# mstksg/tensor-ops

Hardware: AMD Instinct MI355X
Metric: gradTOp steps/sec (ffLayer MNIST 784->256->10) + gmul TFLOP/s vs roofline (higher is better)
Workload: dtype f32

## Files before the change

tensor-ops_amd/csrc/gemm_small.hip:

```cpp
#include "common.hpp"

#include <type_traits>

namespace to {

typedef float f32x16 __attribute__((ext_vector_type(16)));

template <class S>
struct SmallArgsT {
  const S* A;
  const S* B;
  S* C;
  const S* Cin;
  int M, N, K;
  long a_sm, a_sk, b_sk, b_sn, c_sm;
  long a_sb, b_sb, c_sb;
  int a_vec, b_vec;
  unsigned a_bytes, b_bytes;
  int tiles_n;
  int tiles_m;
  int tile_order;
  int kper;
  S alpha, beta;
  const S* bias;
// ... 26 lines not shown
template <class G>
__device__ __forceinline__ void tile_of(const G& g, int bid, int& tile_m, int& tile_n) {
  if (g.tile_order) {
    const int T = g.tiles_m * g.tiles_n, x = bid & 7, q = T >> 3, r = T & 7;
    bid = (x < r ? x * (q + 1) : r * (q + 1) + (x - r) * q) + (bid >> 3);
  }
  if (g.tile_order == 2) {
    tile_n = bid / g.tiles_m;
    tile_m = bid - tile_n * g.tiles_m;
  } else {
    tile_m = bid / g.tiles_n;
    tile_n = bid - tile_m * g.tiles_n;
  }
}

__device__ __forceinline__ float tanh_s(float x) { return tanhf(x); }
__device__ __forceinline__ double tanh_s(double x) { return tanh(x); }
__device__ __forceinline__ float exp_s(float x) { return expf(x); }
__device__ __forceinline__ double exp_s(double x) { return exp(x); }
__device__ __forceinline__ float log_s(float x) { return logf(x); }
__device__ __forceinline__ double log_s(double x) { return log(x); }
__device__ __forceinline__ float max_s(float a, float b) { return fmaxf(a, b); }
__device__ __forceinline__ double max_s(double a, double b) { return fmax(a, b); }

template <class S, int AMODE, int BMODE, int NW, int TS, int ONESHOT = 0, bool EXT = false, int PARTS = 0, bool STAG = false>
__device__ __forceinline__ void gemm_small_body(const SmallArgsT<S>& g, const int bid, const long bz, S* ext_lds = nullptr,
                                                const int tid_in = -1) {
  constexpr int ES = (int)sizeof(S);
  static_assert(ES == 4 || TS == 16, "the fp64 matrix instruction is 16x16x4");
  constexpr int KG = (TS == 32) ? 2 : 4;
  constexpr int NR = (TS == 32) ? 16 : 4;
  constexpr int CK = 4 * KG;
  typedef S accv __attribute__((ext_vector_type(NR)));
  S (*red)[NR][64];
  S (*rsum)[64];
  S* dzs;
  if constexpr (EXT) {
    red = reinterpret_cast<S (*)[NR][64]>(ext_lds);
    rsum = reinterpret_cast<S (*)[64]>(ext_lds + NW * NR * 64);
    dzs = ext_lds + NW * NR * 64 + NW * 64;
  } else {
    __shared__ S red_s[NW][NR][64];
    __shared__ S rsum_s[NW][64];
    __shared__ S dzs_s[TS == 16 ? 16 * 17 : 1];
    red = red_s;
    rsum = rsum_s;
    dzs = dzs_s;
  }
  const int tid = tid_in >= 0 ? tid_in : (int)threadIdx.x, lane = tid & 63, wave = tid >> 6;
  const int l31 = lane & (TS - 1), half = lane / TS;
#ifdef TOPS_AB_KNOBS
  const bool stamp_on = g.dbg && bid == 0 && tid == 0;
#endif
  SM_STAMP(0);
  int tile_m, tile_n;
// ... 95 lines not shown
  };
  auto mma_part = [&](auto part) {
    constexpr int p = decltype(part)::value;
#pragma unroll
    for (int c = p * CP; c < (p + 1) * CP; ++c) {
#pragma unroll
      for (int j = 0; j < 4; ++j) {
        if constexpr (ES == 8) acc = __builtin_amdgcn_mfma_f64_16x16x4f64(a0[c][j], b0[c][j], acc, 0, 0, 0);
        else if constexpr (TS == 32) acc = __builtin_amdgcn_mfma_f32_32x32x2f32(a0[c][j], b0[c][j], acc, 0, 0, 0);
        else acc = __builtin_amdgcn_mfma_f32_16x16x4f32(a0[c][j], b0[c][j], acc, 0, 0, 0);
      }
      __builtin_amdgcn_sched_barrier(0);
#pragma unroll
      for (int j = 0; j < 4; ++j) asum += a0[c][j];
      __builtin_amdgcn_sched_barrier(0);
    }
  };
  auto row16 = [&](int kg, int r) { return ES == 8 ? kg + 4 * r : 4 * kg + r; };
  constexpr int NRW = (NR + NW - 1) / NW;
  S* Cb = g.C + bz * g.c_sb;
  const S* Ci = g.Cin ? g.Cin + bz * g.c_sb : nullptr;
  const S* Hd = g.dact ? g.dact + bz * g.c_sb : nullptr;
  S pf_ci[NRW], pf_hd[NRW], pf_bias = S(0);
  {
    const long col = (long)tile_n * TS + l31;
    if (g.bias && col < g.N) pf_bias = g.bias[col];
#pragma unroll
    for (int i = 0; i < NRW; ++i) {
      const int r = wave + i * NW;
      const int lrow = (TS == 32) ? (r & 3) + 8 * (r >> 2) + 4 * half : row16(half, r);
      const long row = (long)tile_m * TS + lrow;
      const bool ok = r < NR && row < g.M && col < g.N;
      pf_ci[i] = (Ci && ok) ? Ci[row * g.c_sm + col] : S(0);
      pf_hd[i] = (Hd && ok) ? Hd[row * g.c_sm + col] : S(0);
    }
  }
  constexpr int SK = CK * ST;
  SM_STAMP(1);
  if constexpr (ONESHOT) {
    if constexpr (PARTS == 0) {
      if (kbeg < kend) {
        load_stage(a0, b0, kbeg);
#ifdef TOPS_AB_KNOBS
        if (stamp_on) { SM_STAMP(2); __builtin_amdgcn_s_waitcnt(0x0F70); SM_STAMP(3); }
#endif
        mma_stage(a0, b0);
      }
    } else if (kbeg < kend) {
      if constexpr (STAG) {
        const int lvl = __builtin_amdgcn_readfirstlane(wave) >> 2;
        if (lvl == 0) __builtin_amdgcn_s_setprio(3);
        else if (lvl == 1) __builtin_amdgcn_s_setprio(2);
        else if (lvl == 2) __builtin_amdgcn_s_setprio(1);
      }
      load_part(std::integral_constant<int, 0>{}, kbeg);
      auto stage = [&](auto part) {
        constexpr int p = decltype(part)::value;
// ... 10 lines not shown
      if constexpr (PARTS > 2) stage(std::integral_constant<int, 2>{});
      if constexpr (PARTS > 3) stage(std::integral_constant<int, 3>{});
      if constexpr (PARTS > 4) {
        stage(std::integral_constant<int, 4>{});
        stage(std::integral_constant<int, 5>{});
        stage(std::integral_constant<int, 6>{});
        stage(std::integral_constant<int, 7>{});
      }
      static_assert(PARTS == 1 || PARTS == 2 || PARTS == 4 || PARTS == 8, "one, two, four or eight parts");
    }
  } else {
    S a1[ST][4], b1[ST][4];
    if (kbeg < kend) load_stage(a0, b0, kbeg);
    for (int k0 = kbeg; k0 < kend; k0 += 2 * SK) {
      if (k0 + SK < kend) load_stage(a1, b1, k0 + SK);
      mma_stage(a0, b0);
      if (k0 + SK < kend) {
        if (k0 + 2 * SK < kend) load_stage(a0, b0, k0 + 2 * SK);
        mma_stage(a1, b1);
      }
    }
  }

  S tl_bw[2][4], tl_hv[2][4];
  if constexpr (TS == 16) {
    if (g.loss_rows && g.tail_out) {
      const int l15 = lane & 15, kg = lane >> 4;
      const int ntiles = (g.tail_n + 15) / 16;
#pragma unroll
      for (int u = 0; u < 2; ++u) {
        const int t = wave + u * NW;
        const long col = (long)t * 16 + l15;
        const bool cv = t < ntiles && col < g.tail_n;
#pragma unroll
        for (int st = 0; st < 4; ++st) {
          const int k = 4 * st + kg;
          tl_bw[u][st] = (cv && k < g.N) ? g.tail_w[(long)k * g.tail_n + col] : S(0);
        }
#pragma unroll
        for (int r = 0; r < 4; ++r) {
          const long row = (long)tile_m * 16 + row16(kg, r);
          tl_hv[u][r] = (cv && row < g.M) ? g.tail_h[row * g.tail_n + col] : S(0);
        }
      }
    }
  }
#pragma unroll
  for (int r = 0; r < NR; ++r) red[wave][r][lane] = acc[r];
  rsum[wave][lane] = asum;
  SM_STAMP(4);
  __syncthreads();
  SM_STAMP(5);
  if (g.rowsum && tile_n == 0 && wave == 0 && lane < TS) {
    S v = S(0);
#pragma unroll
    for (int w = 0; w < NW; ++w)
#pragma unroll
      for (int q = 0; q < KG; ++q) v += rsum[w][lane + q * TS];
    const long row = (long)tile_m * TS + lane;
    if (row < g.M) g.rowsum[bz * g.M + row] = g.rowsum_acc ? g.rowsum_in[bz * g.M + row] + g.rowsum_alpha * v : v;
  }
#pragma unroll
  for (int i = 0; i < NRW; ++i) {
    const int r = wave + i * NW;
    if (r >= NR) break;
    S v = S(0);
#pragma unroll
    for (int w = 0; w < NW; ++w) v += red[w][r][lane];
    const int lrow = (TS == 32) ? (r & 3) + 8 * (r >> 2) + 4 * half : row16(half, r);
    const long row = (long)tile_m * TS + lrow;
    const long col = (long)tile_n * TS + l31;
    if constexpr (TS == 16) {
      if (g.loss_rows) {
        const bool valid = row < g.M && col < g.N;
        v = v * g.alpha + pf_bias;
        const S t = valid ? g.target[row * g.c_sm + col] : S(0);
        auto sum16 = [](S x) {
#pragma unroll
          for (int off = 8; off > 0; off >>= 1) x += __shfl_xor(x, off, 64);
          return x;
        };
        S out, l;
        if (g.loss_rows == 1) {
          S mx = valid ? v : S(-INFINITY);
#pragma unroll
          for (int off = 8; off > 0; off >>= 1) mx = max_s(mx, __shfl_xor(mx, off, 64));
          const S e = valid ? exp_s(v - mx) : S(0);
          const S se = sum16(e), sy = sum16(t);
          const S pr = e / se;
          out = pr * sy - t;
          l = valid ? -t * log_s(pr) : S(0);
        } else {
          const S sg = S(1) / (S(1) + exp_s(-v));
          const S e = t - sg;
          out = S(-2) * e * sg * (S(1) - sg);
          l = valid ? e * e : S(0);
        }
        if (valid) Cb[row * g.c_sm + col] = out;
        if (g.tail_out) dzs[lrow * 17 + l31] = valid ? out : S(0);
        if (g.loss_out) {
          l = sum16(l);
          if (l31 == 0 && row < g.M) g.loss_out[row] = l;
        }
        continue;
      }
    }
    if (row < g.M && col < g.N) {
      v *= g.alpha;
      if (Ci) v += g.beta * pf_ci[i];
      v += pf_bias;
      if (g.act == 1) v = S(1) / (S(1) + exp_s(-v));
      else if (g.act == 2) v = tanh_s(v);
      if (Hd) {
        const S h = pf_hd[i];
        v *= g.dact_kind ? S(1) - h * h : h * (S(1) - h);
      }
      Cb[row * g.c_sm + col] = v;
    }
  }
  SM_STAMP(6);
  if constexpr (TS == 16) {
    if (g.loss_rows && g.tail_out) {
      __syncthreads();
      typedef S acc4 __attribute__((ext_vector_type(4)));
      const int l15 = lane & 15, kg = lane >> 4;
      const int ntiles = (g.tail_n + 15) / 16;
      acc4 acc2[2];
#pragma unroll
      for (int u = 0; u < 2; ++u)
#pragma unroll
        for (int r = 0; r < 4; ++r) acc2[u][r] = S(0);
#pragma unroll
      for (int st = 0; st < 4; ++st) {
        if (4 * st < g.N) {
          const S a = dzs[l15 * 17 + 4 * st + kg];
#pragma unroll
          for (int u = 0; u < 2; ++u) {
            if constexpr (ES == 8) acc2[u] = __builtin_amdgcn_mfma_f64_16x16x4f64(a, tl_bw[u][st], acc2[u], 0, 0, 0);
            else acc2[u] = __builtin_amdgcn_mfma_f32_16x16x4f32(a, tl_bw[u][st], acc2[u], 0, 0, 0);
          }
        }
      }
#pragma unroll
      for (int u = 0; u < 2; ++u) {
        const int t = wave + u * NW;
        const long col = (long)t * 16 + l15;
#pragma unroll
        for (int r = 0; r < 4; ++r) {
          const long row = (long)tile_m * 16 + row16(kg, r);
          if (t < ntiles && row < g.M && col < g.tail_n)
            g.tail_out[row * g.tail_n + col] = acc2[u][r] * tl_hv[u][r] * (S(1) - tl_hv[u][r]);
        }
      }
      SM_STAMP(7);
    }
  }
#ifdef TOPS_AB_KNOBS
  if (stamp_on) { __builtin_amdgcn_s_waitcnt(0); SM_STAMP(8); }
#endif
}

template <class S, int AMODE, int BMODE, int NW, int TS, int ONESHOT = 0>
__global__ __launch_bounds__(NW * 64) void gemm_small_kernel(SmallArgsT<S> g) {
  gemm_small_body<S, AMODE, BMODE, NW, TS, ONESHOT>(g, (int)blockIdx.x, (long)blockIdx.z);
}

template <class S, int A1, int B1, int NW1, int TS1, int OS1, int A2, int B2, int NW2, int TS2, int OS2, int P1 = 0, bool STAG1 = false>
__global__ __launch_bounds__((NW1 > NW2 ? NW1 : NW2) * 64) void gemm_small_pair_kernel(SmallArgsT<S> g1,
                                                                                         SmallArgsT<S> g2, int n1) {
  if ((int)blockIdx.x < n1) {
    if (NW1 < NW2 && (int)(threadIdx.x >> 6) >= NW1) return;
    gemm_small_body<S, A1, B1, NW1, TS1, OS1, false, P1, STAG1>(g1, (int)blockIdx.x, 0);
  } else {
    if (NW2 < NW1 && (int)(threadIdx.x >> 6) >= NW2) return;
    gemm_small_body<S, A2, B2, NW2, TS2, OS2>(g2, (int)blockIdx.x - n1, 0);
  }
}

struct ChainSync {
  unsigned* ctr;
  int* status;
  long long timeout;
  int dev;
};

__device__ __forceinline__ bool chain_barrier(const ChainSync& cs, int which, unsigned epoch) {
  __shared__ int ok;
  if (cs.dev == 1) {
    __syncthreads();
    return true;
  }
  if (cs.dev != 2) __builtin_amdgcn_fence(__ATOMIC_RELEASE, "agent");
  if (threadIdx.x == 0) ok = 1;
  __syncthreads();
  unsigned* flags = cs.ctr + which * 256;
  if (threadIdx.x == 0) __hip_atomic_store(flags + blockIdx.x, epoch, __ATOMIC_RELEASE, __HIP_MEMORY_SCOPE_AGENT);
  if (threadIdx.x < gridDim.x) {
    const long long t0 = wall_clock64();
// ... 316 lines not shown
  const int tiles_m = (int)((p.M + TS - 1) / TS);
  g.tiles_n = (int)((p.N + TS - 1) / TS);
  g.tiles_m = tiles_m;
  g.tile_order = pick_tile_order(p, TS, g.tiles_m, g.tiles_n);
  dim3 grid(tiles_m * g.tiles_n, 1, (unsigned)p.batch), block(NW * 64);
  switch (amode * 2 + bmode) {
    case 0: launch_k((gemm_small_kernel<S, 0, 0, NW, TS, ONESHOT>), grid, block, 0, s, g); break;
    case 1: launch_k((gemm_small_kernel<S, 0, 1, NW, TS, ONESHOT>), grid, block, 0, s, g); break;
    case 2: launch_k((gemm_small_kernel<S, 1, 0, NW, TS, ONESHOT>), grid, block, 0, s, g); break;
    default: launch_k((gemm_small_kernel<S, 1, 1, NW, TS, ONESHOT>), grid, block, 0, s, g); break;
  }
}

#ifdef TOPS_AB_KNOBS
static long long* small_stamps(int which) {
  static const int want = [] { const char* e = ab_getenv("TOPS_SMALL_STAMPS"); return e ? atoi(e) : 0; }();
  if (!want || want != which) return nullptr;
  static long long* buf = [] {
    long long* p = nullptr;
    if (hipHostMalloc(&p, 16 * sizeof(long long), hipHostMallocMapped) != hipSuccess) return (long long*)nullptr;
    for (int i = 0; i < 16; ++i) p[i] = 0;
    static long long* keep = p;
    atexit([] {
      static const char* names[9] = {"entry", "set-up done", "operand batch issued", "operand batch landed", "MFMAs done, partial in LDS",
                                     "all partials there (barrier)", "reduced + epilogue / loss head, stores issued", "tail done", "stores acknowledged"};
      std::fprintf(stderr, "[small stamps %d] tile 0, thread 0, us since its workgroup began:", want);
      for (int i = 1; i < 9; ++i)
        if (keep[i]) std::fprintf(stderr, "\n  %6.2f  %s", (keep[i] - keep[0]) * 0.01, names[i]);
      std::fprintf(stderr, "\n");
    });
    return p;
  }();
  long long* dev = nullptr;
  if (buf && hipHostGetDevicePointer(reinterpret_cast<void**>(&dev), buf, 0) != hipSuccess) dev = nullptr;
  return dev;
}
#endif

struct SmallPlan {
  int ts, nw, os;
  int amode, bmode;
  bool f64_t32;
};

template <class S>
static SmallPlan plan_small(const GemmProblem& p, SmallArgsT<S>& g) {
  constexpr bool F64 = sizeof(S) == 8;
  g = SmallArgsT<S>{};
  g.A = (const S*)p.A; g.B = (const S*)p.B; g.C = (S*)p.C;
  g.Cin = (p.beta != 0.0) ? (const S*)p.Cin : nullptr;
// ... 344 lines not shown
```

tensor-ops_amd/csrc/gemm_t32.hip:

```cpp
#include <cstdio>
#include <type_traits>

#include "common.hpp"

namespace to {

typedef float f32x16 __attribute__((ext_vector_type(16)));
typedef float f32x4 __attribute__((ext_vector_type(4)));

struct T32Args {
  const float* A;
  const float* B;
  float* C;
  const float* Cin;
  const float* bias;
  const float* dact;
  float* rowsum;
  const float* rowsum_in;
  unsigned long long* dbg;
  long a_sx, b_sx;
  long c_sm;
  int M, N, K;
  int tiles_m, tiles_n;
  int gm, gn;
  int act, dact_kind;
  int rowsum_acc;
  int pd;
  float alpha, beta;
  float rowsum_alpha;
};

__device__ __attribute__((aligned(16))) float g_t32_zero[4] = {0.f, 0.f, 0.f, 0.f};

constexpr int T32_BK = 32, T32_NS = 2, T32_NW = 4;
constexpr int T32_CTR = 4096;
constexpr int T32_STAGE = 2 * 32 * T32_BK;
constexpr int T32_WAVE = T32_NS * T32_STAGE;

__device__ __forceinline__ bool t32_tile_of(int tiles_m, int tiles_n, int gm, int gn, int bid, int& tm, int& tn) {
  const int x = bid & 7, local = bid >> 3, xm = x / gn, xn = x - xm * gn;
  const int r0 = tiles_m * xm / gm, r1 = tiles_m * (xm + 1) / gm, c0 = tiles_n * xn / gn, c1 = tiles_n * (xn + 1) / gn;
  const int w = c1 - c0;
  if (w <= 0 || local >= (r1 - r0) * w) return false;
  tm = r0 + local / w;
  tn = c0 + local - (local / w) * w;
  return true;
}

__device__ __forceinline__ int t32_key(int x) { return (x >> 1) & 7; }

template <bool AKC, bool BKC, bool ARAG = false, bool WT = false, int NW = T32_NW, int NS = T32_NS, bool EARLY = false>
__device__ __forceinline__ int gemm_t32_body(const T32Args& g, const int bid, float* smem) {
  constexpr int WAVE_F = NS * T32_STAGE;
  static_assert(WAVE_F >= 1024 + 64, "a wave's stage memory holds its partial tile and its row sums");
  static_assert(!ARAG || !AKC, "the dword form is for a row-contiguous A");
  constexpr int NA = ARAG ? 16 : 4, PER = NA + 4;
  const int tid = threadIdx.x, lane = tid & 63;
  const int wave = __builtin_amdgcn_readfirstlane(tid >> 6);
  const int l31 = lane & 31, half = lane >> 5;
  unsigned long long* const dbg = (g.dbg && tid == 0 && (bid == 0 || bid == (int)gridDim.x - 1)) ? g.dbg + (bid == 0 ? 0 : 8) : nullptr;
  auto stamp = [&](int i) { if (dbg) dbg[i] = __builtin_amdgcn_s_memrealtime(); };
  int tile_m, tile_n;
  if (!t32_tile_of(g.tiles_m, g.tiles_n, g.gm, g.gn, bid, tile_m, tile_n)) return -1;
  stamp(0);
  const int m0 = tile_m * 32, n0 = tile_n * 32;

  const int erow = tid >> 3, ec4 = (tid & 7) * 4;
  const long grow = m0 + erow, gcol = n0 + ec4;
  const bool evalid = (NW == 4 || tid < 256) && grow < g.M && gcol < g.N;
  f32x4 pf_ci = {0.f, 0.f, 0.f, 0.f}, pf_hd = {0.f, 0.f, 0.f, 0.f}, pf_bias = {0.f, 0.f, 0.f, 0.f};
  auto prefetch_epilogue = [&] {
    if (evalid) {
      if (g.Cin) pf_ci = *reinterpret_cast<const f32x4*>(g.Cin + grow * g.c_sm + gcol);
      if (g.dact) pf_hd = *reinterpret_cast<const f32x4*>(g.dact + grow * g.c_sm + gcol);
      if (g.bias) pf_bias = *reinterpret_cast<const f32x4*>(g.bias + gcol);
    }
  };
  if constexpr (!EARLY) prefetch_epilogue();

  const int U = (g.K + 15) / 16;
  const int k0 = (int)((long)U * wave / NW) * 16;
  int k1 = (int)((long)U * (wave + 1) / NW) * 16;
  if (k1 > g.K) k1 = g.K;
  const int nC = k1 > k0 ? (k1 - k0 + T32_BK - 1) / T32_BK : 0;

  typedef __attribute__((address_space(3))) void* lptr_t;
  float* wsm = smem + wave * WAVE_F;
  const unsigned lds_w = __builtin_amdgcn_readfirstlane((unsigned)(unsigned long)(lptr_t)wsm);

  const int lr = lane >> 3, ls = lane & 7;
  unsigned oa[4], ob[4];
  bool xa_ok = true, xb_ok = true;
#pragma unroll
  for (int p = 0; p < 4; ++p) {
    if constexpr (AKC) {
      long x = m0 + 8 * p + lr;
      if (x >= g.M) x = g.M - 1;
      oa[p] = (unsigned)((x * g.a_sx + 4 * (ls ^ t32_key(8 * p + lr))) * 4);
    } else {
      oa[p] = (unsigned)(((long)(8 * p + lr) * g.a_sx + m0 + 4 * ls) * 4);
    }
    if constexpr (BKC) {
      long x = n0 + 8 * p + lr;
      if (x >= g.N) x = g.N - 1;
      ob[p] = (unsigned)((x * g.b_sx + 4 * (ls ^ t32_key(8 * p + lr))) * 4);
    } else {
      ob[p] = (unsigned)(((long)(8 * p + lr) * g.b_sx + n0 + 4 * ls) * 4);
    }
  }
  if constexpr (!AKC) xa_ok = m0 + 4 * ls + 3 < g.M;
  if constexpr (!BKC) xb_ok = n0 + 4 * ls + 3 < g.N;
  const bool interior = !ARAG && (AKC || m0 + 32 <= g.M) && (BKC || n0 + 32 <= g.N);
  const long step_a = AKC ? T32_BK * 4L : T32_BK * g.a_sx * 4L, step_b = BKC ? T32_BK * 4L : T32_BK * g.b_sx * 4L;
  const char* sa = reinterpret_cast<const char*>(g.A) + (AKC ? (long)k0 * 4 : (long)k0 * g.a_sx * 4);
  const char* sb = reinterpret_cast<const char*>(g.B) + (BKC ? (long)k0 * 4 : (long)k0 * g.b_sx * 4);

#define T32_DMA(OFF, BASE) asm volatile("global_load_lds_dwordx4 %0, %1 offset:0" ::"v"(OFF), "s"(BASE) : "memory")
#define T32_DMA_V(PTR) asm volatile("global_load_lds_dwordx4 %0, off offset:0" ::"v"(PTR) : "memory")
  const long a_sx_l = g.a_sx;
  const int M_l = g.M;
  auto issue = [&, a_sx_l, M_l](int c) {
    const int seq = c;
    const int kc = k0 + c * T32_BK;
    const unsigned st = lds_w + (unsigned)(seq % NS) * (T32_STAGE * 4);
    const char* ba = sa + (long)c * step_a;
    const char* bb = sb + (long)c * step_b;
    const bool full = kc + T32_BK <= k1;
    if (full && interior) {
#pragma unroll
      for (int p = 0; p < 4; ++p) {
        asm volatile("s_mov_b32 m0, %0\n\ts_nop 0" ::"s"(st + p * 1024) : "memory");
        T32_DMA(oa[p], ba);
      }
#pragma unroll
      for (int p = 0; p < 4; ++p) {
        asm volatile("s_mov_b32 m0, %0\n\ts_nop 0" ::"s"(st + 4096 + p * 1024) : "memory");
        T32_DMA(ob[p], bb);
      }
    } else {
      const char* zero = reinterpret_cast<const char*>(g_t32_zero);
      if constexpr (ARAG) {
#pragma unroll
        for (int e = 0; e < 16; ++e) {
          const int kl = 2 * e + half;
          const bool ok = kc + kl < k1 && m0 + l31 < M_l;
          const char* src = ok ? ba + ((long)kl * a_sx_l + m0 + l31) * 4 : zero;
          asm volatile("s_mov_b32 m0, %0\n\ts_nop 0" ::"s"(st + e * 256) : "memory");
          asm volatile("global_load_lds_dword %0, off offset:0" ::"v"(src) : "memory");
        }
      } else {
#pragma unroll
        for (int p = 0; p < 4; ++p) {
          const bool ok = AKC ? (kc + 4 * (ls ^ t32_key(8 * p + lr)) < k1) : (kc + 8 * p + lr < k1 && xa_ok);
          const char* src = ok ? ba + oa[p] : zero;
          asm volatile("s_mov_b32 m0, %0\n\ts_nop 0" ::"s"(st + p * 1024) : "memory");
          T32_DMA_V(src);
        }
      }
#pragma unroll
      for (int p = 0; p < 4; ++p) {
        const bool ok = BKC ? (kc + 4 * (ls ^ t32_key(8 * p + lr)) < k1) : (kc + 8 * p + lr < k1 && xb_ok);
        const char* src = ok ? bb + ob[p] : zero;
        asm volatile("s_mov_b32 m0, %0\n\ts_nop 0" ::"s"(st + 4096 + p * 1024) : "memory");
        T32_DMA_V(src);
      }
    }
  };
#undef T32_DMA
#undef T32_DMA_V

  f32x16 acc;
#pragma unroll
  for (int r = 0; r < 16; ++r) acc[r] = 0.f;
  float asum = 0.f;
  const bool want_rs = g.rowsum != nullptr && tile_n == 0;

  const int PD = g.pd < NS ? g.pd : NS;
  const int pro = nC < PD ? nC : PD;
  if constexpr (EARLY) {
    if (pro > 0) issue(0);
    __builtin_amdgcn_sched_barrier(0);
    prefetch_epilogue();
    __builtin_amdgcn_sched_barrier(0);
    for (int c = 1; c < pro; ++c) issue(c);
  } else {
    for (int c = 0; c < pro; ++c) issue(c);
  }
  stamp(1);

  auto wait_landed = [&](int c) {
    const int newer = (nC - 1 - c) < (PD - 1) ? (nC - 1 - c) : (PD - 1);
    static_assert(3 * PER <= 63, "vmcnt is six bits");
    if (newer >= 3) asm volatile("s_waitcnt vmcnt(%0)" ::"n"(3 * PER) : "memory");
    else if (newer == 2) asm volatile("s_waitcnt vmcnt(%0)" ::"n"(2 * PER) : "memory");
    else if (newer == 1) asm volatile("s_waitcnt vmcnt(%0)" ::"n"(PER) : "memory");
    else asm volatile("s_waitcnt vmcnt(0)" ::: "memory");
  };
  auto steps_of = [&](int c) { return (k1 - (k0 + c * T32_BK)) > 16 ? 4 : 2; };
  auto read_frags = [&](int c, float (&fa)[16], float (&fb)[16]) {
    const float* sp = wsm + (c % NS) * T32_STAGE;
    const int nI = steps_of(c);
#pragma unroll
    for (int i = 0; i < 4; ++i) {
      if (i < nI) {
        if constexpr (AKC) {
          const f32x4 v = *reinterpret_cast<const f32x4*>(sp + l31 * 32 + 4 * ((2 * i + half) ^ t32_key(l31)));
          fa[4 * i] = v.x; fa[4 * i + 1] = v.y; fa[4 * i + 2] = v.z; fa[4 * i + 3] = v.w;
        } else {
#pragma unroll
          for (int j = 0; j < 4; ++j) fa[4 * i + j] = sp[(4 * (2 * i + half) + j) * 32 + l31];
        }
        if constexpr (BKC) {
          const f32x4 v = *reinterpret_cast<const f32x4*>(sp + 1024 + l31 * 32 + 4 * ((2 * i + half) ^ t32_key(l31)));
          fb[4 * i] = v.x; fb[4 * i + 1] = v.y; fb[4 * i + 2] = v.z; fb[4 * i + 3] = v.w;
        } else {
#pragma unroll
          for (int j = 0; j < 4; ++j) fb[4 * i + j] = sp[1024 + (4 * (2 * i + half) + j) * 32 + l31];
        }
      }
    }
  };
  auto mma = [&](int c, const float (&fa)[16], const float (&fb)[16]) {
    const int nI = steps_of(c);
#pragma unroll
    for (int i = 0; i < 4; ++i) {
      if (i < nI) {
#pragma unroll
        for (int j = 0; j < 4; ++j) {
          acc = __builtin_amdgcn_mfma_f32_32x32x2f32(fa[4 * i + j], fb[4 * i + j], acc, 0, 0, 0);
          if (want_rs) asum += fa[4 * i + j];
        }
      }
    }
  };
  float fa[16], fb[16];
  for (int c = 0; c < nC; ++c) {
    wait_landed(c);
    if (c == 0) stamp(2);
    read_frags(c, fa, fb);
    asm volatile("s_waitcnt lgkmcnt(0)" ::: "memory");
    __builtin_amdgcn_sched_barrier(0);
    if (c + PD < nC) issue(c + PD);
    __builtin_amdgcn_sched_barrier(0);
    mma(c, fa, fb);
  }
  asm volatile("s_waitcnt vmcnt(0)" ::: "memory");
  stamp(3);

#pragma unroll
  for (int r = 0; r < 16; ++r) wsm[((r & 3) + 8 * (r >> 2) + 4 * half) * 32 + l31] = acc[r];
  if (want_rs) wsm[1024 + lane] = asum;
  __syncthreads();
  stamp(4);
  f32x4 s = {0.f, 0.f, 0.f, 0.f};
  if (NW == 4 || tid < 256) {
    s = *reinterpret_cast<const f32x4*>(smem + erow * 32 + ec4);
#pragma unroll
    for (int w = 1; w < NW; ++w) s += *reinterpret_cast<const f32x4*>(smem + w * WAVE_F + erow * 32 + ec4);
// ... 147 lines not shown
  if (hd) hd[3] = __builtin_amdgcn_s_memrealtime();
  if (h.tail_out) {
    f32x4 a = {0.f, 0.f, 0.f, 0.f};
#pragma unroll
    for (int n = 0; n < 16; ++n)
      if (n < h.N2) {
        const float d = __shfl(out_l, n, 64);
        a += w4[n] * d;
      }
    if (rv) *reinterpret_cast<f32x4*>(h.tail_out + grow * 256 + 4 * lane) = a * h4 * (1.f - h4);
  }
  if (hd) hd[4] = __builtin_amdgcn_s_memrealtime();
  __syncthreads();
  if (tid == 0) {
    unsigned* leave = h.ctr + T32_CTR + tile_m;
    const unsigned seen = __hip_atomic_fetch_add(leave, 1u, __ATOMIC_RELAXED, __HIP_MEMORY_SCOPE_AGENT);
    if (seen == (unsigned)(g.tiles_n - 1)) {
      __hip_atomic_store(h.ctr + tile_m, 0u, __ATOMIC_RELAXED, __HIP_MEMORY_SCOPE_AGENT);
      __hip_atomic_store(leave, 0u, __ATOMIC_RELAXED, __HIP_MEMORY_SCOPE_AGENT);
    }
  }
}

template <bool AKC, bool BKC, int NW = T32_NW, int NS = T32_NS, bool EARLY = false>
__global__ __launch_bounds__(NW * 64) void gemm_t32_kernel(T32Args g) {
  extern __shared__ __attribute__((aligned(1024))) float t32_smem[];
  gemm_t32_body<AKC, BKC, false, false, NW, NS, EARLY>(g, (int)blockIdx.x, t32_smem);
}

template <bool ARAG2>
__global__ __launch_bounds__(256) void gemm_t32_pair_kernel(T32Args g1, T32Args g2, int n1) {
  extern __shared__ __attribute__((aligned(1024))) float t32_smem[];
  if ((int)blockIdx.x < n1) gemm_t32_body<false, false, false>(g1, (int)blockIdx.x, t32_smem);
  else gemm_t32_body<false, false, ARAG2>(g2, (int)blockIdx.x - n1, t32_smem);
}

static bool t32_fill(const GemmProblem& p, T32Args& g, bool& akc, bool& bkc, bool allow_ragged_a = false, bool* ragged_a = nullptr) {
  if (p.dtype != TO_F32 || p.batch != 1 || p.reduce_batch) return false;
  if (p.loss_rows || p.tail_out || p.loss_out) return false;
  akc = p.a_sk == 1 && p.K > 1;
  bkc = p.b_sk == 1 && p.K > 1;
  if (!akc && p.a_sm != 1) return false;
  if (!bkc && p.b_sn != 1) return false;
  if (p.K % 4 != 0 || p.N % 4 != 0) return false;
  const bool rag = !akc && (p.M % 4 != 0 || p.a_sk % 4 != 0 || (reinterpret_cast<uintptr_t>(p.A) & 15u));
  if (ragged_a) *ragged_a = rag;
  if (rag && !allow_ragged_a) return false;
  if (akc && p.a_sm % 4 != 0) return false;
  if (bkc && p.b_sn % 4 != 0) return false;
  if (!bkc && p.b_sk % 4 != 0) return false;
// ... 58 lines not shown
bool gemm_t32_applicable(const GemmProblem& p) {
  static const int enable = [] { const char* e = ab_getenv("TOPS_GEMM_T32"); return e ? atoi(e) : 1; }();
  if (!enable) return false;
  T32Args g;
  bool akc, bkc;
  if (!t32_fill(p, g, akc, bkc)) return false;
  const long tiles = (long)g.tiles_m * g.tiles_n;
  static const long max_tiles = [] { const char* e = ab_getenv("TOPS_T32_MAXTILES"); return e ? atol(e) : 512L; }();
  return tiles >= 96 && tiles <= max_tiles && p.K >= 256 && p.K <= 8192;
}

bool launch_gemm_t32_pair(const GemmProblem& p1, const GemmProblem& p2, hipStream_t s);

static long t32_grid(const T32Args& g) {
  const long rm = (g.tiles_m + g.gm - 1) / g.gm, rn = (g.tiles_n + g.gn - 1) / g.gn;
  return 8 * rm * rn;
}

static void t32_attr(const void* k) { TO_HIP(hipFuncSetAttribute(k, hipFuncAttributeMaxDynamicSharedMemorySize, T32_NW * T32_WAVE * 4)); }

constexpr int T32_W8_DEFAULT = 1;
constexpr int T32_W8_NS = 1;
constexpr bool T32_EARLY = true;

template <int NW, int NS, bool EARLY>
static void t32_launch_nw(const T32Args& g, bool akc, bool bkc, hipStream_t s) {
  constexpr size_t lds = (size_t)NW * NS * T32_STAGE * 4;
  static bool attr = false;
  if (!attr) {
    TO_HIP(hipFuncSetAttribute(reinterpret_cast<const void*>(gemm_t32_kernel<true, true, NW, NS, EARLY>), hipFuncAttributeMaxDynamicSharedMemorySize, (int)lds));
    TO_HIP(hipFuncSetAttribute(reinterpret_cast<const void*>(gemm_t32_kernel<true, false, NW, NS, EARLY>), hipFuncAttributeMaxDynamicSharedMemorySize, (int)lds));
    TO_HIP(hipFuncSetAttribute(reinterpret_cast<const void*>(gemm_t32_kernel<false, true, NW, NS, EARLY>), hipFuncAttributeMaxDynamicSharedMemorySize, (int)lds));
    TO_HIP(hipFuncSetAttribute(reinterpret_cast<const void*>(gemm_t32_kernel<false, false, NW, NS, EARLY>), hipFuncAttributeMaxDynamicSharedMemorySize, (int)lds));
    attr = true;
  }
  const dim3 grid((unsigned)t32_grid(g)), block(NW * 64);
  if (akc && bkc) launch_k((gemm_t32_kernel<true, true, NW, NS, EARLY>), grid, block, lds, s, g);
  else if (akc) launch_k((gemm_t32_kernel<true, false, NW, NS, EARLY>), grid, block, lds, s, g);
  else if (bkc) launch_k((gemm_t32_kernel<false, true, NW, NS, EARLY>), grid, block, lds, s, g);
  else launch_k((gemm_t32_kernel<false, false, NW, NS, EARLY>), grid, block, lds, s, g);
}

void launch_gemm_t32(const GemmProblem& p, hipStream_t s) {
  T32Args g;
  bool akc, bkc;
  TO_CHECK(t32_fill(p, g, akc, bkc), TO_ERR_STATE, "launch_gemm_t32: not applicable");
  static const int cus = [] { hipDeviceProp_t pr; int d = 0; return (hipGetDevice(&d) == hipSuccess && hipGetDeviceProperties(&pr, d) == hipSuccess) ? pr.multiProcessorCount : 0; }();
  static const int waves = [] { const char* e = ab_getenv("TOPS_T32_WAVES"); return e ? atoi(e) : (T32_W8_DEFAULT ? 8 : 4); }();
  const bool w8 = waves == 8 && t32_grid(g) <= cus;
#ifdef TOPS_AB_KNOBS
  static const int w8_ns = [] { const char* e = ab_getenv("TOPS_T32_W8_NS"); return e ? atoi(e) : T32_W8_NS; }();
  static const int early = [] { const char* e = ab_getenv("TOPS_T32_EARLY"); return e ? atoi(e) : (int)T32_EARLY; }();
  switch ((w8 ? (w8_ns == 1 ? 2 : 4) : 0) + (early ? 1 : 0)) {
    case 0: t32_launch_nw<T32_NW, T32_NS, false>(g, akc, bkc, s); break;
    case 1: t32_launch_nw<T32_NW, T32_NS, true>(g, akc, bkc, s); break;
    case 2: t32_launch_nw<8, 1, false>(g, akc, bkc, s); break;
    case 3: t32_launch_nw<8, 1, true>(g, akc, bkc, s); break;
    case 4: t32_launch_nw<8, 2, false>(g, akc, bkc, s); break;
    default: t32_launch_nw<8, 2, true>(g, akc, bkc, s); break;
  }
#else
  if (w8) t32_launch_nw<8, T32_W8_NS, T32_EARLY>(g, akc, bkc, s);
  else t32_launch_nw<T32_NW, T32_NS, T32_EARLY>(g, akc, bkc, s);
#endif
  TO_HIP(hipGetLastError());
  count_launch();
}

static unsigned* g_t32_ctr = nullptr;
static int *g_t32_status = nullptr, *g_t32_status_dev = nullptr;
static bool g_t32_head_off = false;
void gemm_t32_init() {
  if (g_t32_ctr) return;
  if (hipMalloc(&g_t32_ctr, 2 * T32_CTR * sizeof(unsigned)) != hipSuccess || hipMemset(g_t32_ctr, 0, 2 * T32_CTR * sizeof(unsigned)) != hipSuccess) {
    (void)hipGetLastError();
    g_t32_ctr = nullptr;
    return;
  }
  if (hipHostMalloc(&g_t32_status, sizeof(int), hipHostMallocMapped) == hipSuccess) {
    *g_t32_status = 0;
    if (hipHostGetDevicePointer(reinterpret_cast<void**>(&g_t32_status_dev), g_t32_status, 0) != hipSuccess) g_t32_status_dev = nullptr;
  }
  (void)hipGetLastError();
}
int gemm_t32_take_failure() {
// ... 80 lines not shown
```

Before: 41720.

## Prefetch loss-head operands early, use DPP reductions, add 3-unit K-chunk plans

In the small GEMM loss-head path, the target, rowsum input and tail operands are now loaded before the MFMA loop so their latency overlaps the matrix work. The 16-lane shuffles become DPP row rotates, and the head's stores and loss reduction are deferred until after the tail GEMM. Separately, the eight-wave t32 kernel gains chunk plans that group three 16-wide K units per trip when a wave's share is odd, with extra LDS stage space, which cuts the number of load-wait-compute rounds. Plan 1 is the default, so LDS use per wave grows and register pressure rises from the larger fragment arrays.

```diff
diff --git a/tensor-ops_amd/csrc/gemm_small.hip b/tensor-ops_amd/csrc/gemm_small.hip
--- a/tensor-ops_amd/csrc/gemm_small.hip
+++ b/tensor-ops_amd/csrc/gemm_small.hip
@@ -72,8 +72,14 @@
 __device__ __forceinline__ double log_s(double x) { return log(x); }
 __device__ __forceinline__ float max_s(float a, float b) { return fmaxf(a, b); }
 __device__ __forceinline__ double max_s(double a, double b) { return fmax(a, b); }
-
-template <class S, int AMODE, int BMODE, int NW, int TS, int ONESHOT = 0, bool EXT = false, int PARTS = 0, bool STAG = false>
+template <int N>
+__device__ __forceinline__ float dpp_ror(float x) {
+  return __uint_as_float((unsigned)__builtin_amdgcn_update_dpp(0, (int)__float_as_uint(x), 0x120 + N, 0xf, 0xf, false));
+}
+template <int N>
+__device__ __forceinline__ double dpp_ror(double x) { return x; }
+
+template <class S, int AMODE, int BMODE, int NW, int TS, int ONESHOT = 0, bool EXT = false, int PARTS = 0, bool STAG = false, bool HEAD = true>
 __device__ __forceinline__ void gemm_small_body(const SmallArgsT<S>& g, const int bid, const long bz, S* ext_lds = nullptr,
                                                 const int tid_in = -1) {
   constexpr int ES = (int)sizeof(S);
@@ -81,6 +87,7 @@
   constexpr int KG = (TS == 32) ? 2 : 4;
   constexpr int NR = (TS == 32) ? 16 : 4;
   constexpr int CK = 4 * KG;
+  constexpr bool LH = HEAD && TS == 16;
   typedef S accv __attribute__((ext_vector_type(NR)));
   S (*red)[NR][64];
   S (*rsum)[64];
@@ -222,6 +229,7 @@
   const S* Ci = g.Cin ? g.Cin + bz * g.c_sb : nullptr;
   const S* Hd = g.dact ? g.dact + bz * g.c_sb : nullptr;
   S pf_ci[NRW], pf_hd[NRW], pf_bias = S(0);
+  S pf_tg[NRW];
   {
     const long col = (long)tile_n * TS + l31;
     if (g.bias && col < g.N) pf_bias = g.bias[col];
@@ -233,6 +241,38 @@
       const bool ok = r < NR && row < g.M && col < g.N;
       pf_ci[i] = (Ci && ok) ? Ci[row * g.c_sm + col] : S(0);
       pf_hd[i] = (Hd && ok) ? Hd[row * g.c_sm + col] : S(0);
+      pf_tg[i] = S(0);
+      if constexpr (LH) {
+        if (g.loss_rows && ok) pf_tg[i] = g.target[row * g.c_sm + col];
+      }
+    }
+  }
+  const bool rs_lane = g.rowsum && tile_n == 0 && wave == 0 && lane < TS && (long)tile_m * TS + lane < g.M;
+  S pf_rs = S(0);
+  if constexpr (TS == 16) {
+    if (rs_lane && g.rowsum_acc) pf_rs = g.rowsum_in[bz * g.M + (long)tile_m * TS + lane];
+  }
+  S tl_bw[2][4], tl_hv[2][4];
+  if constexpr (LH) {
+    if (g.loss_rows && g.tail_out) {
+      const int l15 = lane & 15, kg = lane >> 4;
+      const int ntiles = (g.tail_n + 15) / 16;
+#pragma unroll
+      for (int u = 0; u < 2; ++u) {
+        const int t = wave + u * NW;
+        const long col = (long)t * 16 + l15;
+        const bool cv = t < ntiles && col < g.tail_n;
+#pragma unroll
+        for (int st = 0; st < 4; ++st) {
+          const int k = 4 * st + kg;
+          tl_bw[u][st] = (cv && k < g.N) ? g.tail_w[(long)k * g.tail_n + col] : S(0);
+        }
+#pragma unroll
+        for (int r = 0; r < 4; ++r) {
+          const long row = (long)tile_m * 16 + row16(kg, r);
+          tl_hv[u][r] = (cv && row < g.M) ? g.tail_h[row * g.tail_n + col] : S(0);
+        }
+      }
     }
   }
   constexpr int SK = CK * ST;
@@ -289,44 +329,64 @@
     }
   }
 
-  S tl_bw[2][4], tl_hv[2][4];
-  if constexpr (TS == 16) {
-    if (g.loss_rows && g.tail_out) {
-      const int l15 = lane & 15, kg = lane >> 4;
-      const int ntiles = (g.tail_n + 15) / 16;
-#pragma unroll
-      for (int u = 0; u < 2; ++u) {
-        const int t = wave + u * NW;
-        const long col = (long)t * 16 + l15;
-        const bool cv = t < ntiles && col < g.tail_n;
-#pragma unroll
-        for (int st = 0; st < 4; ++st) {
-          const int k = 4 * st + kg;
-          tl_bw[u][st] = (cv && k < g.N) ? g.tail_w[(long)k * g.tail_n + col] : S(0);
-        }
-#pragma unroll
-        for (int r = 0; r < 4; ++r) {
-          const long row = (long)tile_m * 16 + row16(kg, r);
-          tl_hv[u][r] = (cv && row < g.M) ? g.tail_h[row * g.tail_n + col] : S(0);
-        }
-      }
-    }
-  }
 #pragma unroll
   for (int r = 0; r < NR; ++r) red[wave][r][lane] = acc[r];
   rsum[wave][lane] = asum;
   SM_STAMP(4);
   __syncthreads();
   SM_STAMP(5);
-  if (g.rowsum && tile_n == 0 && wave == 0 && lane < TS) {
+  auto rowsum_out = [&] {
+    if (!rs_lane) return;
     S v = S(0);
 #pragma unroll
     for (int w = 0; w < NW; ++w)
 #pragma unroll
       for (int q = 0; q < KG; ++q) v += rsum[w][lane + q * TS];
     const long row = (long)tile_m * TS + lane;
-    if (row < g.M) g.rowsum[bz * g.M + row] = g.rowsum_acc ? g.rowsum_in[bz * g.M + row] + g.rowsum_alpha * v : v;
-  }
+    if constexpr (TS != 16) {
+      if (g.rowsum_acc) pf_rs = g.rowsum_in[bz * g.M + row];
+    }
+    g.rowsum[bz * g.M + row] = g.rowsum_acc ? pf_rs + g.rowsum_alpha * v : v;
+  };
+  if constexpr (TS != 16) rowsum_out();
+  auto sum16 = [](S x) {
+    if constexpr (ES == 4) {
+      x += dpp_ror<8>(x); x += dpp_ror<4>(x); x += dpp_ror<2>(x); x += dpp_ror<1>(x);
+    } else {
+#pragma unroll
+      for (int off = 8; off > 0; off >>= 1) x += __shfl_xor(x, off, 64);
+    }
+    return x;
+  };
+  auto max16 = [](S x) {
+    if constexpr (ES == 4) {
+      x = max_s(x, dpp_ror<8>(x)); x = max_s(x, dpp_ror<4>(x)); x = max_s(x, dpp_ror<2>(x)); x = max_s(x, dpp_ror<1>(x));
+    } else {
+#pragma unroll
+      for (int off = 8; off > 0; off >>= 1) x = max_s(x, __shfl_xor(x, off, 64));
+    }
+    return x;
+  };
+  S hd_out[NRW], hd_l[NRW];
+#pragma unroll
+  for (int i = 0; i < NRW; ++i) hd_out[i] = hd_l[i] = S(0);
+  auto head_out = [&] {
+#pragma unroll
+    for (int i = 0; i < NRW; ++i) {
+      const int r = wave + i * NW;
+      if (r >= NR) break;
+      const long row = (long)tile_m * TS + row16(half, r);
+      const long col = (long)tile_n * TS + l31;
+      const bool valid = row < g.M && col < g.N;
+      if (valid) Cb[row * g.c_sm + col] = hd_out[i];
+      if (g.loss_out) {
+        S l = hd_l[i];
+        if (g.loss_rows == 1) l = -pf_tg[i] * log_s(l);
+        l = sum16(valid ? l : S(0));
+        if (l31 == 0 && row < g.M) g.loss_out[row] = l;
+      }
+    }
+  };
 #pragma unroll
   for (int i = 0; i < NRW; ++i) {
     const int r = wave + i * NW;
@@ -337,38 +397,27 @@
     const int lrow = (TS == 32) ? (r & 3) + 8 * (r >> 2) + 4 * half : row16(half, r);
     const long row = (long)tile_m * TS + lrow;
     const long col = (long)tile_n * TS + l31;
-    if constexpr (TS == 16) {
+    if constexpr (LH) {
       if (g.loss_rows) {
         const bool valid = row < g.M && col < g.N;
         v = v * g.alpha + pf_bias;
-        const S t = valid ? g.target[row * g.c_sm + col] : S(0);
-        auto sum16 = [](S x) {
-#pragma unroll
-          for (int off = 8; off > 0; off >>= 1) x += __shfl_xor(x, off, 64);
-          return x;
-        };
-        S out, l;
+        const S t = pf_tg[i];
+        S out;
         if (g.loss_rows == 1) {
-          S mx = valid ? v : S(-INFINITY);
-#pragma unroll
-          for (int off = 8; off > 0; off >>= 1) mx = max_s(mx, __shfl_xor(mx, off, 64));
+          const S mx = max16(valid ? v : S(-INFINITY));
           const S e = valid ? exp_s(v - mx) : S(0);
           const S se = sum16(e), sy = sum16(t);
           const S pr = e / se;
           out = pr * sy - t;
-          l = valid ? -t * log_s(pr) : S(0);
+          hd_l[i] = pr;
         } else {
           const S sg = S(1) / (S(1) + exp_s(-v));
           const S e = t - sg;
           out = S(-2) * e * sg * (S(1) - sg);
-          l = valid ? e * e : S(0);
+          hd_l[i] = e * e;
         }
-        if (valid) Cb[row * g.c_sm + col] = out;
+        hd_out[i] = out;
         if (g.tail_out) dzs[lrow * 17 + l31] = valid ? out : S(0);
-        if (g.loss_out) {
-          l = sum16(l);
-          if (l31 == 0 && row < g.M) g.loss_out[row] = l;
-        }
         continue;
       }
     }
@@ -386,7 +435,8 @@
     }
   }
   SM_STAMP(6);
-  if constexpr (TS == 16) {
+  if constexpr (LH) {
+    if (g.loss_rows && !g.tail_out) head_out();
     if (g.loss_rows && g.tail_out) {
       __syncthreads();
       typedef S acc4 __attribute__((ext_vector_type(4)));
@@ -408,6 +458,8 @@
           }
         }
       }
+      __builtin_amdgcn_sched_barrier(0);
+      SM_STAMP(9);
 #pragma unroll
       for (int u = 0; u < 2; ++u) {
         const int t = wave + u * NW;
@@ -419,9 +471,12 @@
             g.tail_out[row * g.tail_n + col] = acc2[u][r] * tl_hv[u][r] * (S(1) - tl_hv[u][r]);
         }
       }
+      __builtin_amdgcn_sched_barrier(0);
+      head_out();
       SM_STAMP(7);
     }
   }
+  if constexpr (TS == 16) rowsum_out();
 #ifdef TOPS_AB_KNOBS
   if (stamp_on) { __builtin_amdgcn_s_waitcnt(0); SM_STAMP(8); }
 #endif
@@ -437,10 +492,10 @@
                                                                                          SmallArgsT<S> g2, int n1) {
   if ((int)blockIdx.x < n1) {
     if (NW1 < NW2 && (int)(threadIdx.x >> 6) >= NW1) return;
-    gemm_small_body<S, A1, B1, NW1, TS1, OS1, false, P1, STAG1>(g1, (int)blockIdx.x, 0);
+    gemm_small_body<S, A1, B1, NW1, TS1, OS1, false, P1, STAG1, false>(g1, (int)blockIdx.x, 0);
   } else {
     if (NW2 < NW1 && (int)(threadIdx.x >> 6) >= NW2) return;
-    gemm_small_body<S, A2, B2, NW2, TS2, OS2>(g2, (int)blockIdx.x - n1, 0);
+    gemm_small_body<S, A2, B2, NW2, TS2, OS2, false, 0, false, false>(g2, (int)blockIdx.x - n1, 0);
   }
 }
 
@@ -803,10 +858,11 @@
     for (int i = 0; i < 16; ++i) p[i] = 0;
     static long long* keep = p;
     atexit([] {
-      static const char* names[9] = {"entry", "set-up done", "operand batch issued", "operand batch landed", "MFMAs done, partial in LDS",
-                                     "all partials there (barrier)", "reduced + epilogue / loss head, stores issued", "tail done", "stores acknowledged"};
+      static const char* names[10] = {"entry", "set-up done", "operand batch issued", "operand batch landed", "MFMAs done, partial in LDS",
+                                      "all partials there (barrier)", "reduced + epilogue / loss head done", "tail done", "stores acknowledged",
+                                      "tail's MFMAs issued"};
       std::fprintf(stderr, "[small stamps %d] tile 0, thread 0, us since its workgroup began:", want);
-      for (int i = 1; i < 9; ++i)
+      for (int i : {1, 2, 3, 4, 5, 6, 9, 7, 8})
         if (keep[i]) std::fprintf(stderr, "\n  %6.2f  %s", (keep[i] - keep[0]) * 0.01, names[i]);
       std::fprintf(stderr, "\n");
     });
diff --git a/tensor-ops_amd/csrc/gemm_t32.hip b/tensor-ops_amd/csrc/gemm_t32.hip
--- a/tensor-ops_amd/csrc/gemm_t32.hip
+++ b/tensor-ops_amd/csrc/gemm_t32.hip
@@ -37,6 +37,25 @@
 constexpr int T32_STAGE = 2 * 32 * T32_BK;
 constexpr int T32_WAVE = T32_NS * T32_STAGE;
 
+constexpr int T32_PLANS = 4;
+__host__ __device__ constexpr int t32_stage_floats(int plan) { return plan == 0 ? T32_STAGE : T32_STAGE + 2 * 32 * 16; }
+__host__ __device__ constexpr int t32_plan_trips(int plan, int n) {
+  return n <= 0 ? 0 : plan == 0 ? (n + 1) / 2 : plan == 3 ? (n + 2) / 3 : (n < 2 ? 1 : n / 2);
+}
+__host__ __device__ constexpr void t32_plan_chunk(int plan, int n, int c, int& start, int& size) {
+  if (plan == 3) {
+    start = 3 * c;
+    size = n - start < 3 ? n - start : 3;
+  } else if (plan == 2 && (n & 1) && n >= 3) {
+    start = c ? 2 * c + 1 : 0;
+    size = c ? 2 : 3;
+  } else {
+    start = 2 * c;
+    size = n - start < 2 ? n - start : 2;
+    if (plan == 1 && n - start == 3) size = 3;
+  }
+}
+
 __device__ __forceinline__ bool t32_tile_of(int tiles_m, int tiles_n, int gm, int gn, int bid, int& tm, int& tn) {
   const int x = bid & 7, local = bid >> 3, xm = x / gn, xn = x - xm * gn;
   const int r0 = tiles_m * xm / gm, r1 = tiles_m * (xm + 1) / gm, c0 = tiles_n * xn / gn, c1 = tiles_n * (xn + 1) / gn;
@@ -48,12 +67,16 @@
 }
 
 __device__ __forceinline__ int t32_key(int x) { return (x >> 1) & 7; }
-
-template <bool AKC, bool BKC, bool ARAG = false, bool WT = false, int NW = T32_NW, int NS = T32_NS, bool EARLY = false>
+__device__ __forceinline__ int t32_key3(int x) { return (x >> 2) & 3; }
+
+template <bool AKC, bool BKC, bool ARAG = false, bool WT = false, int NW = T32_NW, int NS = T32_NS, bool EARLY = false, int PLAN = 0>
 __device__ __forceinline__ int gemm_t32_body(const T32Args& g, const int bid, float* smem) {
-  constexpr int WAVE_F = NS * T32_STAGE;
+  constexpr int STAGE_F = t32_stage_floats(PLAN);
+  constexpr int WAVE_F = NS * STAGE_F;
   static_assert(WAVE_F >= 1024 + 64, "a wave's stage memory holds its partial tile and its row sums");
+  static_assert((size_t)8 * WAVE_F * 4 <= 160 * 1024, "eight waves' stages fit a CU's LDS");
   static_assert(!ARAG || !AKC, "the dword form is for a row-contiguous A");
+  static_assert(PLAN == 0 || (NS == 1 && !ARAG), "3-unit chunks: one stage a wave (the wait is vmcnt(0)), no dword form");
   constexpr int NA = ARAG ? 16 : 4, PER = NA + 4;
   const int tid = threadIdx.x, lane = tid & 63;
   const int wave = __builtin_amdgcn_readfirstlane(tid >> 6);
@@ -82,7 +105,8 @@
   const int k0 = (int)((long)U * wave / NW) * 16;
   int k1 = (int)((long)U * (wave + 1) / NW) * 16;
   if (k1 > g.K) k1 = g.K;
-  const int nC = k1 > k0 ? (k1 - k0 + T32_BK - 1) / T32_BK : 0;
+  const int nU = k1 > k0 ? (k1 - k0 + 15) / 16 : 0;
+  const int nC = t32_plan_trips(PLAN, nU);
 
   typedef __attribute__((address_space(3))) void* lptr_t;
   float* wsm = smem + wave * WAVE_F;
@@ -108,10 +132,31 @@
       ob[p] = (unsigned)(((long)(8 * p + lr) * g.b_sx + n0 + 4 * ls) * 4);
     }
   }
+  unsigned oa3[2] = {0u, 0u}, ob3[2] = {0u, 0u};
+  const int lr3 = lane >> 2, ls3 = lane & 3;
+  if constexpr (PLAN != 0) {
+#pragma unroll
+    for (int p = 0; p < 2; ++p) {
+      if constexpr (AKC) {
+        long x = m0 + 16 * p + lr3;
+        if (x >= g.M) x = g.M - 1;
+        oa3[p] = (unsigned)((x * g.a_sx + 4 * (ls3 ^ t32_key3(16 * p + lr3))) * 4);
+      } else {
+        oa3[p] = oa[p];
+      }
+      if constexpr (BKC) {
+        long x = n0 + 16 * p + lr3;
+        if (x >= g.N) x = g.N - 1;
+        ob3[p] = (unsigned)((x * g.b_sx + 4 * (ls3 ^ t32_key3(16 * p + lr3))) * 4);
+      } else {
+        ob3[p] = ob[p];
+      }
+    }
+  }
   if constexpr (!AKC) xa_ok = m0 + 4 * ls + 3 < g.M;
   if constexpr (!BKC) xb_ok = n0 + 4 * ls + 3 < g.N;
   const bool interior = !ARAG && (AKC || m0 + 32 <= g.M) && (BKC || n0 + 32 <= g.N);
-  const long step_a = AKC ? T32_BK * 4L : T32_BK * g.a_sx * 4L, step_b = BKC ? T32_BK * 4L : T32_BK * g.b_sx * 4L;
+  const long step_a = AKC ? 16 * 4L : 16 * g.a_sx * 4L, step_b = BKC ? 16 * 4L : 16 * g.b_sx * 4L;
   const char* sa = reinterpret_cast<const char*>(g.A) + (AKC ? (long)k0 * 4 : (long)k0 * g.a_sx * 4);
   const char* sb = reinterpret_cast<const char*>(g.B) + (BKC ? (long)k0 * 4 : (long)k0 * g.b_sx * 4);
 
@@ -119,12 +164,18 @@
 #define T32_DMA_V(PTR) asm volatile("global_load_lds_dwordx4 %0, off offset:0" ::"v"(PTR) : "memory")
   const long a_sx_l = g.a_sx;
   const int M_l = g.M;
+  auto chunk_of = [&](int c, int& kc, int& sz) {
+    int us;
+    t32_plan_chunk(PLAN, nU, c, us, sz);
+    kc = k0 + 16 * us;
+    return us;
+  };
   auto issue = [&, a_sx_l, M_l](int c) {
-    const int seq = c;
-    const int kc = k0 + c * T32_BK;
-    const unsigned st = lds_w + (unsigned)(seq % NS) * (T32_STAGE * 4);
-    const char* ba = sa + (long)c * step_a;
-    const char* bb = sb + (long)c * step_b;
+    int kc, sz;
+    const int us = chunk_of(c, kc, sz);
+    const unsigned st = lds_w + (unsigned)(c % NS) * (STAGE_F * 4);
+    const char* ba = sa + (long)us * step_a;
+    const char* bb = sb + (long)us * step_b;
     const bool full = kc + T32_BK <= k1;
     if (full && interior) {
 #pragma unroll
@@ -163,6 +214,41 @@
         const char* src = ok ? bb + ob[p] : zero;
         asm volatile("s_mov_b32 m0, %0\n\ts_nop 0" ::"s"(st + 4096 + p * 1024) : "memory");
         T32_DMA_V(src);
+      }
+    }
+    if constexpr (PLAN != 0) {
+      if (sz == 3) {
+        const int kx = kc + T32_BK;
+        const char* ba3 = ba + 2 * step_a;
+        const char* bb3 = bb + 2 * step_b;
+        if (kx + 16 <= k1 && interior) {
+#pragma unroll
+          for (int p = 0; p < 2; ++p) {
+            asm volatile("s_mov_b32 m0, %0\n\ts_nop 0" ::"s"(st + 8192 + p * 1024) : "memory");
+            T32_DMA(oa3[p], ba3);
+          }
+#pragma unroll
+          for (int p = 0; p < 2; ++p) {
+            asm volatile("s_mov_b32 m0, %0\n\ts_nop 0" ::"s"(st + 10240 + p * 1024) : "memory");
+            T32_DMA(ob3[p], bb3);
+          }
+        } else {
+          const char* zero = reinterpret_cast<const char*>(g_t32_zero);
+#pragma unroll
+          for (int p = 0; p < 2; ++p) {
+            const bool ok = AKC ? (kx + 4 * (ls3 ^ t32_key3(16 * p + lr3)) < k1) : (kx + 8 * p + lr < k1 && xa_ok);
+            const char* src = ok ? ba3 + oa3[p] : zero;
+            asm volatile("s_mov_b32 m0, %0\n\ts_nop 0" ::"s"(st + 8192 + p * 1024) : "memory");
+            T32_DMA_V(src);
+          }
+#pragma unroll
+          for (int p = 0; p < 2; ++p) {
+            const bool ok = BKC ? (kx + 4 * (ls3 ^ t32_key3(16 * p + lr3)) < k1) : (kx + 8 * p + lr < k1 && xb_ok);
+            const char* src = ok ? bb3 + ob3[p] : zero;
+            asm volatile("s_mov_b32 m0, %0\n\ts_nop 0" ::"s"(st + 10240 + p * 1024) : "memory");
+            T32_DMA_V(src);
+          }
+        }
       }
     }
   };
@@ -196,9 +282,10 @@
     else if (newer == 1) asm volatile("s_waitcnt vmcnt(%0)" ::"n"(PER) : "memory");
     else asm volatile("s_waitcnt vmcnt(0)" ::: "memory");
   };
-  auto steps_of = [&](int c) { return (k1 - (k0 + c * T32_BK)) > 16 ? 4 : 2; };
-  auto read_frags = [&](int c, float (&fa)[16], float (&fb)[16]) {
-    const float* sp = wsm + (c % NS) * T32_STAGE;
+  constexpr int NI = PLAN != 0 ? 6 : 4, NF = 4 * NI;
+  auto steps_of = [&](int c) { int kc, sz; chunk_of(c, kc, sz); return 2 * sz; };
+  auto read_frags = [&](int c, float (&fa)[NF], float (&fb)[NF]) {
+    const float* sp = wsm + (c % NS) * STAGE_F;
     const int nI = steps_of(c);
 #pragma unroll
     for (int i = 0; i < 4; ++i) {
@@ -219,11 +306,33 @@
         }
       }
     }
+    if constexpr (PLAN != 0) {
+      if (nI == 6) {
+#pragma unroll
+        for (int i = 4; i < 6; ++i) {
+          const int q = 2 * (i - 4) + half;
+          if constexpr (AKC) {
+            const f32x4 v = *reinterpret_cast<const f32x4*>(sp + 2048 + l31 * 16 + 4 * (q ^ t32_key3(l31)));
+            fa[4 * i] = v.x; fa[4 * i + 1] = v.y; fa[4 * i + 2] = v.z; fa[4 * i + 3] = v.w;
+          } else {
+#pragma unroll
+            for (int j = 0; j < 4; ++j) fa[4 * i + j] = sp[2048 + (4 * q + j) * 32 + l31];
+          }
+          if constexpr (BKC) {
+            const f32x4 v = *reinterpret_cast<const f32x4*>(sp + 2560 + l31 * 16 + 4 * (q ^ t32_key3(l31)));
+            fb[4 * i] = v.x; fb[4 * i + 1] = v.y; fb[4 * i + 2] = v.z; fb[4 * i + 3] = v.w;
+          } else {
+#pragma unroll
+            for (int j = 0; j < 4; ++j) fb[4 * i + j] = sp[2560 + (4 * q + j) * 32 + l31];
+          }
+        }
+      }
+    }
   };
-  auto mma = [&](int c, const float (&fa)[16], const float (&fb)[16]) {
+  auto mma = [&](int c, const float (&fa)[NF], const float (&fb)[NF]) {
     const int nI = steps_of(c);
 #pragma unroll
-    for (int i = 0; i < 4; ++i) {
+    for (int i = 0; i < NI; ++i) {
       if (i < nI) {
 #pragma unroll
         for (int j = 0; j < 4; ++j) {
@@ -233,7 +342,7 @@
       }
     }
   };
-  float fa[16], fb[16];
+  float fa[NF], fb[NF];
   for (int c = 0; c < nC; ++c) {
     wait_landed(c);
     if (c == 0) stamp(2);
@@ -427,10 +536,10 @@
   }
 }
 
-template <bool AKC, bool BKC, int NW = T32_NW, int NS = T32_NS, bool EARLY = false>
+template <bool AKC, bool BKC, int NW = T32_NW, int NS = T32_NS, bool EARLY = false, int PLAN = 0>
 __global__ __launch_bounds__(NW * 64) void gemm_t32_kernel(T32Args g) {
   extern __shared__ __attribute__((aligned(1024))) float t32_smem[];
-  gemm_t32_body<AKC, BKC, false, false, NW, NS, EARLY>(g, (int)blockIdx.x, t32_smem);
+  gemm_t32_body<AKC, BKC, false, false, NW, NS, EARLY, PLAN>(g, (int)blockIdx.x, t32_smem);
 }
 
 template <bool ARAG2>
@@ -535,24 +644,40 @@
 constexpr int T32_W8_DEFAULT = 1;
 constexpr int T32_W8_NS = 1;
 constexpr bool T32_EARLY = true;
-
-template <int NW, int NS, bool EARLY>
+constexpr int T32_W8_PLAN = 1;
+
+template <int NW, int NS, bool EARLY, int PLAN = 0>
 static void t32_launch_nw(const T32Args& g, bool akc, bool bkc, hipStream_t s) {
-  constexpr size_t lds = (size_t)NW * NS * T32_STAGE * 4;
+  constexpr size_t lds = (size_t)NW * NS * t32_stage_floats(PLAN) * 4;
   static bool attr = false;
   if (!attr) {
-    TO_HIP(hipFuncSetAttribute(reinterpret_cast<const void*>(gemm_t32_kernel<true, true, NW, NS, EARLY>), hipFuncAttributeMaxDynamicSharedMemorySize, (int)lds));
-    TO_HIP(hipFuncSetAttribute(reinterpret_cast<const void*>(gemm_t32_kernel<true, false, NW, NS, EARLY>), hipFuncAttributeMaxDynamicSharedMemorySize, (int)lds));
-    TO_HIP(hipFuncSetAttribute(reinterpret_cast<const void*>(gemm_t32_kernel<false, true, NW, NS, EARLY>), hipFuncAttributeMaxDynamicSharedMemorySize, (int)lds));
-    TO_HIP(hipFuncSetAttribute(reinterpret_cast<const void*>(gemm_t32_kernel<false, false, NW, NS, EARLY>), hipFuncAttributeMaxDynamicSharedMemorySize, (int)lds));
+    TO_HIP(hipFuncSetAttribute(reinterpret_cast<const void*>(gemm_t32_kernel<true, true, NW, NS, EARLY, PLAN>), hipFuncAttributeMaxDynamicSharedMemorySize, (int)lds));
+    TO_HIP(hipFuncSetAttribute(reinterpret_cast<const void*>(gemm_t32_kernel<true, false, NW, NS, EARLY, PLAN>), hipFuncAttributeMaxDynamicSharedMemorySize, (int)lds));
+    TO_HIP(hipFuncSetAttribute(reinterpret_cast<const void*>(gemm_t32_kernel<false, true, NW, NS, EARLY, PLAN>), hipFuncAttributeMaxDynamicSharedMemorySize, (int)lds));
+    TO_HIP(hipFuncSetAttribute(reinterpret_cast<const void*>(gemm_t32_kernel<false, false, NW, NS, EARLY, PLAN>), hipFuncAttributeMaxDynamicSharedMemorySize, (int)lds));
     attr = true;
   }
   const dim3 grid((unsigned)t32_grid(g)), block(NW * 64);
-  if (akc && bkc) launch_k((gemm_t32_kernel<true, true, NW, NS, EARLY>), grid, block, lds, s, g);
-  else if (akc) launch_k((gemm_t32_kernel<true, false, NW, NS, EARLY>), grid, block, lds, s, g);
-  else if (bkc) launch_k((gemm_t32_kernel<false, true, NW, NS, EARLY>), grid, block, lds, s, g);
-  else launch_k((gemm_t32_kernel<false, false, NW, NS, EARLY>), grid, block, lds, s, g);
-}
+  if (akc && bkc) launch_k((gemm_t32_kernel<true, true, NW, NS, EARLY, PLAN>), grid, block, lds, s, g);
+  else if (akc) launch_k((gemm_t32_kernel<true, false, NW, NS, EARLY, PLAN>), grid, block, lds, s, g);
+  else if (bkc) launch_k((gemm_t32_kernel<false, true, NW, NS, EARLY, PLAN>), grid, block, lds, s, g);
+  else launch_k((gemm_t32_kernel<false, false, NW, NS, EARLY, PLAN>), grid, block, lds, s, g);
+}
+
+extern "C" __attribute__((visibility("default"))) int to_t32_chunk_plan(int plan, int U, int nw, int wave, int* out, int cap) {
+  if (plan < 0 || plan >= T32_PLANS || U < 0 || nw < 1 || wave < 0 || wave >= nw) return -1;
+  const int u0 = (int)((long)U * wave / nw), u1 = (int)((long)U * (wave + 1) / nw), n = u1 - u0;
+  const int nc = t32_plan_trips(plan, n);
+  if (nc > cap) return -1;
+  for (int c = 0; c < nc; ++c) {
+    int st, sz;
+    t32_plan_chunk(plan, n, c, st, sz);
+    out[2 * c] = u0 + st;
+    out[2 * c + 1] = sz;
+  }
+  return nc;
+}
+extern "C" __attribute__((visibility("default"))) int to_t32_w8_plan() { return T32_W8_PLAN; }
 
 void launch_gemm_t32(const GemmProblem& p, hipStream_t s) {
   T32Args g;
@@ -564,16 +689,23 @@
 #ifdef TOPS_AB_KNOBS
   static const int w8_ns = [] { const char* e = ab_getenv("TOPS_T32_W8_NS"); return e ? atoi(e) : T32_W8_NS; }();
   static const int early = [] { const char* e = ab_getenv("TOPS_T32_EARLY"); return e ? atoi(e) : (int)T32_EARLY; }();
+  static const int plan = [] { const char* e = ab_getenv("TOPS_T32_W8_PLAN"); const int v = e ? atoi(e) : T32_W8_PLAN; return v < 0 || v >= T32_PLANS ? 0 : v; }();
   switch ((w8 ? (w8_ns == 1 ? 2 : 4) : 0) + (early ? 1 : 0)) {
     case 0: t32_launch_nw<T32_NW, T32_NS, false>(g, akc, bkc, s); break;
     case 1: t32_launch_nw<T32_NW, T32_NS, true>(g, akc, bkc, s); break;
     case 2: t32_launch_nw<8, 1, false>(g, akc, bkc, s); break;
-    case 3: t32_launch_nw<8, 1, true>(g, akc, bkc, s); break;
+    case 3:
+      if (plan == 1) t32_launch_nw<8, 1, true, 1>(g, akc, bkc, s);
+      else if (plan == 2) t32_launch_nw<8, 1, true, 2>(g, akc, bkc, s);
+      else if (plan == 3) t32_launch_nw<8, 1, true, 3>(g, akc, bkc, s);
+      else t32_launch_nw<8, 1, true>(g, akc, bkc, s);
+      break;
     case 4: t32_launch_nw<8, 2, false>(g, akc, bkc, s); break;
     default: t32_launch_nw<8, 2, true>(g, akc, bkc, s); break;
   }
 #else
-  if (w8) t32_launch_nw<8, T32_W8_NS, T32_EARLY>(g, akc, bkc, s);
+  static_assert(T32_W8_NS == 1 || T32_W8_PLAN == 0, "the 3-unit chunk plans run one stage a wave");
+  if (w8) t32_launch_nw<8, T32_W8_NS, T32_EARLY, T32_W8_PLAN>(g, akc, bkc, s);
   else t32_launch_nw<T32_NW, T32_NS, T32_EARLY>(g, akc, bkc, s);
 #endif
   TO_HIP(hipGetLastError());
```

After: 41790, median of 6. No clear change (+0.2%).
